# NVlabs/long-video-gan

Hardware: NVIDIA H100
Metric: frames/sec (G+D train step: every convolution and torch_utils.ops call of the forward/backward passes, replayed) (higher is better)
Workload: dtype f32

## Files before the change

include/lvg_ops.h:

```cpp
#ifndef LVG_OPS_H_
#define LVG_OPS_H_

#include <stdint.h>

#ifdef __cplusplus
extern "C" {
#endif

#define LVG_ABI_VERSION 2

#define LVG_OK            0
#define LVG_UNSUPPORTED (-1)
#define LVG_ERR_ARG       1
#define LVG_ERR_CUDA      2

#define LVG_F32 0
#define LVG_F16 1
#define LVG_F64 2

#define LVG_ACT_LINEAR   1
#define LVG_ACT_RELU     2
#define LVG_ACT_LRELU    3
#define LVG_ACT_TANH     4
#define LVG_ACT_SIGMOID  5
// ... 24 lines not shown
                           void* stream);
int64_t lvg_bias_act_codes_bytes(int dtype, int64_t n);

int lvg_upfirdn2d(const void* x, const float* f, void* y, int dtype,
                  const int64_t x_shape[4], const int64_t x_stride[4],
                  const int64_t y_shape[4], const int64_t y_stride[4],
                  int fw, int fh, int64_t f_stride_x, int64_t f_stride_y,
                  int upx, int upy, int downx, int downy, int padx0, int pady0,
                  int flip, float gain, void* stream);

int lvg_upfirdn2d_sep(const void* x, const float* fx, const float* fy, void* y,
                      int dtype, const int64_t x_shape[4], const int64_t x_stride[4],
                      const int64_t y_shape[4], const int64_t y_stride[4],
                      int fw, int fh, int upx, int upy, int downx, int downy,
                      int padx0, int pady0, int flip, float gain, void* stream);

int lvg_filtered_lrelu(const void* x, const float* fu, const float* fd, const void* b,
                       const uint8_t* si, void* y, uint8_t* so, int dtype,
                       const int64_t x_shape[4], const int64_t x_stride[4],
                       const int64_t y_shape[4], const int64_t y_stride[4],
                       int fu_w, int fu_h, int fd_w, int fd_h, int up, int down,
                       int px0, int py0, int s_h, int s_wbytes, int sx, int sy,
                       float gain, float slope, float clamp, int flip,
                       int write_signs, void* stream);

int lvg_filtered_lrelu_supported(int dtype, int fu_w, int fu_h, int fd_w, int fd_h,
                                 int up, int down);

int lvg_filtered_lrelu_act(void* x, const uint8_t* si, uint8_t* so, int dtype,
                           const int64_t x_shape[4], const int64_t x_stride[4],
                           int s_h, int s_wbytes, int sx, int sy, float gain,
                           float slope, float clamp, int write_signs, void* stream);

int lvg_fma(const void* a, const void* b, const void* c, void* out, int dtype,
            int rank, const int64_t shape[6], const int64_t a_stride[6],
            const int64_t b_stride[6], const int64_t c_stride[6], void* stream);

int64_t lvg_convnd_workspace(int dtype, int n, int groups, int cin, int cout, int t, int h, int wd,
                             int kt, int kh, int kw, int pad_t, int pad_h, int pad_w);
int lvg_convnd_fprop(const void* x, const void* w, void* y, int dtype, int n, int groups, int cin, int cout,
                     int t, int h, int wd, int kt, int kh, int kw, int pad_t, int pad_h, int pad_w, int stride,
                     const float* bias, int act, float alpha, float gain, float clamp,
                     void* workspace, int64_t workspace_bytes, void* stream);
int lvg_convnd_dgrad(const void* dy, const void* w, void* dx, int dtype, int n, int groups, int cin, int cout,
                     int t, int h, int wd, int kt, int kh, int kw, int pad_t, int pad_h, int pad_w, int stride,
                     void* workspace, int64_t workspace_bytes, void* stream);
int64_t lvg_convnd_wgrad_workspace(int dtype, int n, int groups, int cin, int cout, int t, int h, int wd,
                                   int kt, int kh, int kw, int pad_t, int pad_h, int pad_w);
int lvg_convnd_wgrad(const void* x, const void* dy, void* dw, int dtype, int n, int groups, int cin, int cout,
                     int t, int h, int wd, int kt, int kh, int kw, int pad_t, int pad_h, int pad_w, int stride,
                     void* workspace, int64_t workspace_bytes, void* stream);
int lvg_convnd_plan(int mode, int dtype, int n, int groups, int cin, int cout, int t, int h, int wd, int kt, int kh, int kw,
                    int pad_t, int pad_h, int pad_w, int stride, int* out, int out_len);
int lvg_convnd_wgrad_plan(int dtype, int n, int groups, int cin, int cout, int t, int h, int wd, int kt, int kh, int kw,
                          int pad_t, int pad_h, int pad_w, int* out, int out_len);
int64_t lvg_convnd_backward_workspace(int dtype, int n, int groups, int cin, int cout, int t, int h, int wd,
                                      int kt, int kh, int kw, int pad_t, int pad_h, int pad_w);
int lvg_convnd_backward(const void* x, const void* dy, const void* w, void* dx, void* dw, int dtype, int n, int groups,
                        int cin, int cout, int t, int h, int wd, int kt, int kh, int kw, int pad_t, int pad_h, int pad_w,
                        int stride, void* workspace, int64_t workspace_bytes, void* stream);

int64_t lvg_modconv_workspace(int dtype, int n, int cin, int cout, int t, int h, int wd, int kt, int kh, int kw,
                              int pad_t, int pad_h, int pad_w);
int lvg_modconv_fprop(const void* x, const void* w, const float* a, const float* d, void* y, int dtype, int n, int cin,
                      int cout, int t, int h, int wd, int kt, int kh, int kw, int pad_t, int pad_h, int pad_w,
                      void* workspace, int64_t workspace_bytes, void* stream);
int lvg_modconv_backward(const void* x, const void* w, const float* a, const float* d, const void* y, const void* dy,
                         void* dx, void* dw, float* da, float* dyy, int dtype, int n, int cin, int cout, int t, int h,
                         int wd, int kt, int kh, int kw, int pad_t, int pad_h, int pad_w, void* workspace,
                         int64_t workspace_bytes, void* stream);

int64_t lvg_fir1d_depthwise_workspace(int groups);
int lvg_fir1d_depthwise(const float* x, const float* w, float* y, int n, int groups, int lin, int k,
                        void* workspace, int64_t workspace_bytes, void* stream);

int lvg_fir3d(const void* x, const float* f, void* y, int dtype, int n, int c, int t_in, int h_in, int w_in, int t_out,
              int h_out, int w_out, int filt_t, int filt_h, int filt_w, int step_t, int step_h, int step_w, int off_t,
              int off_h, int off_w, int fold, void* stream);
int lvg_fir3d_adjoint(const void* x, const float* f, void* y, int dtype, int n, int c, int t_in, int h_in, int w_in,
                      int t_out, int h_out, int w_out, int filt_t, int filt_h, int filt_w, int step_t, int step_h,
                      int step_w, int off_t, int off_h, int off_w, int fold, void* stream);

#define LVG_VIDEO_AUGMENT_LINEAR 1
int64_t lvg_video_augment_workspace(int n, int c, int t_in, int h, int w, int t_out);
int lvg_video_augment(const float* x, const float* params, float* y, void* workspace, int n, int c, int t_in, int h, int w,
                      int t_out, int flags, void* stream);
int lvg_video_augment_adjoint(const float* dy, const float* params, float* dx, void* workspace, int n, int c, int t_in,
                              int h, int w, int t_out, void* stream);

#define LVG_AUGMENT_PIPE_NPAR 23
#define LVG_AUGMENT_PIPE_GEOM 1
#define LVG_AUGMENT_PIPE_LINEAR 2
int64_t lvg_augment_pipe_workspace(int n, int c, int t, int h, int w, int flags);
int lvg_augment_pipe(const float* x, const float* params, const float* filter, int ntaps, const float* noise, float* y, int n,
                     int c, int t, int h, int w, int flags, void* stream);
int lvg_augment_pipe_adjoint(const float* dy, const float* params, const float* filter, int ntaps, float* dx, void* workspace,
                             int n, int c, int t, int h, int w, int flags, void* stream);

int lvg_grad_postprocess(float* g, int64_t n, float scale, float limit, void* stream);

int lvg_adam_step(float* p, float* g, float* m, float* v, float* p_ema, int64_t n, float lr, float beta1, float beta2,
                  float eps, int64_t step, float grad_scale, float grad_limit, int write_grad, float ema_beta, void* stream);

int lvg_lerp(float* a, const float* b, int64_t n, float weight, void* stream);

#ifdef __cplusplus
// ... 4 lines not shown
```

long-video-gan_b200/csrc/conv_igemm.cu:

```cuda

#include <algorithm>
#include <cuda.h>
#include <stdlib.h>
#include <cuda_bf16.h>

#include "common.cuh"
#include "wgmma.cuh"

namespace lvg {
bool pw_supported(int dtype, int groups, int cin, int cout, int kt, int kh, int kw, int pad_t, int pad_h, int pad_w, int stride, int64_t P);
int pw_conv(const float* x, const float* w, float* y, int n, int cin, int cout, int64_t P, int64_t w_sco, int64_t w_sci, cudaStream_t s);
}

namespace lvg {
namespace {

using namespace tc;

constexpr int kBM = 128;
constexpr int kATile = kBM * 16 * 2;
constexpr int kIgemmThreads = 384;
constexpr int kWidths = 16;
constexpr int kMaxStages = 6;
constexpr int kBSlack = 1024;

struct IgemmParams {
    const unsigned char* wp;
    void* y;
    const float* bias;
    int act;
    float alpha, gain, clamp;
    int out_f32;
    int bf16;
    int wgroups, cout, mt, kc;
    int nblk;
    int nimg;
    int lo_blk;
    int to, ho, wo;
    int kt, kh, kw, pad_t, pad_h, pad_w;
    int tt, th, wt, wtb, thb;
    int frame_px;
    int ncols;
    int m64;
    int ncw;
    int a_img;
    int tiles_x, tiles_y, tiles_t;
    int64_t total_tiles;
    int ks;
    int stages;
    int a_resident;
    int a_stage, b_step, b_bytes, b_box, stage_bytes;
    int64_t y_cs;
    int ostride, hos, wos;
    const float* out_scale;
};


__device__ __forceinline__ unsigned short bf16_bits(float v) { return __bfloat16_as_ushort(__float2bfloat16_rn(v)); }
__device__ __forceinline__ float bf16_val(unsigned short b) { return __uint_as_float((uint32_t)b << 16); }

struct PackGeom { int64_t thw_in, thw_out; int ih, iw, oh, ow, dil; const float* scale; };

template <class TIn, bool SPLIT, bool SCALE>
__global__ void __launch_bounds__(256) conv_pack_act_kernel(const TIn* __restrict__ x, uint4* __restrict__ y, int64_t inst, int c,
// ... 546 lines not shown
        const int rc = encode_map(&tm, x8, wd, h, t, inst * g.nblk, wd, (int64_t)h * wd, thw, p.wtb, p.thb, p.tt, 2);
        if (rc) return rc;
    }
    const size_t smem = (size_t)p.stages * p.stage_bytes + 128;
#define LVG_IGEMM_WIDTHS(B, S)                                                                                                     \
    {conv_igemm_kernel<B, 16, S>,  conv_igemm_kernel<B, 32, S>,  conv_igemm_kernel<B, 48, S>,  conv_igemm_kernel<B, 64, S>,        \
     conv_igemm_kernel<B, 80, S>,  conv_igemm_kernel<B, 96, S>,  conv_igemm_kernel<B, 112, S>, conv_igemm_kernel<B, 128, S>,       \
     conv_igemm_kernel<B, 144, S>, conv_igemm_kernel<B, 160, S>, conv_igemm_kernel<B, 176, S>, conv_igemm_kernel<B, 192, S>,       \
     conv_igemm_kernel<B, 208, S>, conv_igemm_kernel<B, 224, S>, conv_igemm_kernel<B, 240, S>, conv_igemm_kernel<B, 256, S>}
    void (*const kerns[2][2][kWidths])(const CUtensorMap, const IgemmParams) = {
        {LVG_IGEMM_WIDTHS(false, false), LVG_IGEMM_WIDTHS(true, false)}, {LVG_IGEMM_WIDTHS(false, true), LVG_IGEMM_WIDTHS(true, true)}};
#undef LVG_IGEMM_WIDTHS
    LVG_REQUIRE(p.ncw % 16 == 0 && p.ncw >= 16 && p.ncw <= 16 * kWidths, "convnd: MMA width %d", p.ncw);
    void (*kern)(const CUtensorMap, const IgemmParams) = kerns[out_scale != nullptr][split][p.ncw / 16 - 1];
    LVG_CUDA(cudaFuncSetAttribute(kern, cudaFuncAttributeMaxDynamicSharedMemorySize, (int)smem));
    const char* cta_env = getenv("LVG_CONV_CTAS");
    const int max_ctas = cta_env ? atoi(cta_env) : num_sms();
    int64_t ctas = p.total_tiles < max_ctas ? p.total_tiles : max_ctas;
    kern<<<(unsigned)ctas, kIgemmThreads, smem, s>>>(tm, p);
    LVG_LAUNCH_CHECK();
    return LVG_OK;
}

bool nd_supported(int dtype, int kt, int kh, int kw)
{
    return (dtype == LVG_F16 || dtype == LVG_F32) && kt >= 1 && kh >= 1 && kw >= 1 && kh * kw <= 9 && kt <= 7;
}

}
}

using namespace lvg;

extern "C" int64_t lvg_convnd_workspace(int dtype, int n, int groups, int cin, int cout, int t, int h, int wd, int kt, int kh, int kw,
                                        int pad_t, int pad_h, int pad_w)
{
    if (!nd_supported(dtype, kt, kh, kw) || n < 1 || groups < 1) return -1;
    const int split = dtype == LVG_F32;
    const int taps = kt * kh * kw;
    const int64_t inst = (int64_t)n * groups;
    const int to = t + 2 * pad_t - kt + 1, ho = h + 2 * pad_h - kh + 1, wo = wd + 2 * pad_w - kw + 1;
    if (to < 1 || ho < 1 || wo < 1) return -1;
    const Geometry a = geometry(split, inst, groups, cin, cout, (int64_t)t * h * wd, taps);
    const Geometry b = geometry(split, inst, groups, cout, cin, (int64_t)to * ho * wo, taps);
    const int64_t fa = a.act_bytes + a.w_bytes, fb = b.act_bytes + b.w_bytes;
    return (fa > fb ? fa : fb) + 1024;
}

extern "C" int lvg_convnd_fprop(const void* x, const void* w, void* y, int dtype, int n, int groups, int cin, int cout, int t, int h, int wd,
                                int kt, int kh, int kw, int pad_t, int pad_h, int pad_w, int stride, const float* bias, int act, float alpha,
                                float gain, float clamp, void* workspace, int64_t workspace_bytes, void* stream)
{
    LVG_REQUIRE(x && w && y, "convnd_fprop: x, w, y must not be NULL");
    if (!bias && act == 0 && gain == 1.f && clamp < 0.f &&
        pw_supported(dtype, groups, cin, cout, kt, kh, kw, pad_t, pad_h, pad_w, stride, (int64_t)t * h * wd))
        return pw_conv((const float*)x, (const float*)w, (float*)y, n, cin, cout, (int64_t)t * h * wd, cin, 1, (cudaStream_t)stream);
    if (!nd_supported(dtype, kt, kh, kw) || n < 1 || pad_t < 0 || pad_h < 0 || pad_w < 0 || stride < 1 || stride > 4) {
        set_error("convnd_fprop: outside the tensor-core kernel's envelope");
        return LVG_UNSUPPORTED;
    }
    const int taps = kt * kh * kw;
    return run_igemm(x, w, y, dtype, n, groups, cin, cout, t, h, wd, kt, kh, kw, pad_t, pad_h, pad_w, (int64_t)cout * cin * taps,
                     (int64_t)cin * taps, taps, 0, bias, act, alpha, gain, clamp, h, wd, 1, stride, nullptr, workspace, workspace_bytes,
                     (cudaStream_t)stream);
}

extern "C" int lvg_convnd_dgrad(const void* dy, const void* w, void* dx, int dtype, int n, int groups, int cin, int cout, int t, int h, int wd,
                                int kt, int kh, int kw, int pad_t, int pad_h, int pad_w, int stride, void* workspace, int64_t workspace_bytes,
                                void* stream)
{
    LVG_REQUIRE(dy && w && dx, "convnd_dgrad: dy, w, dx must not be NULL");
    if (pw_supported(dtype, groups, cin, cout, kt, kh, kw, pad_t, pad_h, pad_w, stride, (int64_t)t * h * wd))
        return pw_conv((const float*)dy, (const float*)w, (float*)dx, n, cout, cin, (int64_t)t * h * wd, 1, cin, (cudaStream_t)stream);
    if (!nd_supported(dtype, kt, kh, kw) || n < 1 || pad_t < 0 || pad_h < 0 || pad_w < 0 || pad_t > kt - 1 || pad_h > kh - 1 || pad_w > kw - 1 ||
        stride < 1 || stride > 4) {
        set_error("convnd_dgrad: outside the tensor-core kernel's envelope");
        return LVG_UNSUPPORTED;
    }
    const int taps = kt * kh * kw;
    const int to = t + 2 * pad_t - kt + 1, ho = h + 2 * pad_h - kh + 1, wo = wd + 2 * pad_w - kw + 1;
    const int hos = (ho - 1) / stride + 1, wos = (wo - 1) / stride + 1;
    return run_igemm(dy, w, dx, dtype, n, groups, cout, cin, to, ho, wo, kt, kh, kw, kt - 1 - pad_t, kh - 1 - pad_h, kw - 1 - pad_w,
                     (int64_t)cout * cin * taps, taps, (int64_t)cin * taps, 1, nullptr, 0, 0.f, 1.f, -1.f, hos, wos, stride, 1, nullptr, workspace,
                     workspace_bytes, (cudaStream_t)stream);
}


namespace lvg {
namespace {

struct WgradV2Params {
    void* dw;
    int out_f32;
    int bf16, split;
    int n, groups, cin, cout;
    int to, ho;
    int kt, kh, kw, pad_t, pad_h, pad_w;
    int nt;
    int nblk_a, nblk_b;
    int lo_a, lo_b;
    int nseg, seg_w[4], seg_x0[4], ps[4];
    int rh;
    int khc;
    int ablk;
    int nsplit;
    int a_bytes, b_bytes, stage_bytes, stages;
    int64_t split_stride;
    int mrows;
    int tail_bytes;
};

struct WgradMaps { CUtensorMap a[4]; CUtensorMap b; };

template <bool BF16, int TAPS, int NT>
__global__ void __launch_bounds__(kIgemmThreads, 1) conv_wgrad_v2_kernel(const __grid_constant__ WgradMaps maps, const WgradV2Params p)
{
    extern __shared__ __align__(128) unsigned char smem_raw[];
    __shared__ uint64_t full_bar[kMaxStages], empty_bar[kMaxStages];
    unsigned char* smem = reinterpret_cast<unsigned char*>((reinterpret_cast<uintptr_t>(smem_raw) + 127) & ~(uintptr_t)127);

    const int warp = threadIdx.x / 32, lane = threadIdx.x % 32;
    const int wg = __shfl_sync(0xffffffffu, (int)threadIdx.x / 128, 0);
    int bx = blockIdx.x;
    const int sp = bx % p.nsplit; bx /= p.nsplit;
    int ky0 = 0;
    if (p.khc == 1) { ky0 = bx % p.kh; bx /= p.kh; }
// ... 278 lines not shown
    {
        const int rc = encode_map(&maps.b, x8, wd, h, t, inst * p.nblk_b, wd, (int64_t)h * wd, thw_b, p.ps[0], p.rh + q.khc - 1, 1, q.nt / 8);
        if (rc) return rc;
    }
    void (*const kern)(const WgradMaps, const WgradV2Params) = wgrad_kernel(q.split, q.khc * kw, q.nt);
    LVG_REQUIRE(kern != nullptr, "convnd_wgrad: no kernel for %d taps x %d columns (split %d)", q.khc * kw, q.nt, q.split);
    LVG_CUDA(cudaFuncSetAttribute(kern, cudaFuncAttributeMaxDynamicSharedMemorySize, (int)smem));
    dim3 grid((unsigned)(q.ntiles * kt * (kh / q.khc) * q.nsplit), (unsigned)q.mt, (unsigned)groups);
    kern<<<grid, kIgemmThreads, smem, s>>>(maps, p);
    LVG_LAUNCH_CHECK();
    if (q.nsplit > 1) {
        int64_t blocks = (q.dw_elems + 255) / 256;
        const int64_t cap = (int64_t)num_sms() * 32;
        if (blocks > cap) blocks = cap;
        if (q.split) conv_wgrad_reduce_kernel<float><<<(unsigned)blocks, 256, 0, s>>>(part, (float*)dw, q.dw_elems, q.nsplit, q.dw_elems);
        else conv_wgrad_reduce_kernel<__half><<<(unsigned)blocks, 256, 0, s>>>(part, (__half*)dw, q.dw_elems, q.nsplit, q.dw_elems);
        LVG_LAUNCH_CHECK();
    }
    return LVG_OK;
}

bool wgrad_in_envelope(int dtype, int n, int groups, int t, int h, int wd, int kt, int kh, int kw, int pad_t, int pad_h, int pad_w, int stride)
{
    const int to = t + 2 * pad_t - kt + 1, ho = h + 2 * pad_h - kh + 1, wo = wd + 2 * pad_w - kw + 1;
    return nd_supported(dtype, kt, kh, kw) && n >= 1 && groups >= 1 && kw <= 3 && pad_t >= 0 && pad_h >= 0 && pad_w >= 0 && to >= 1 && ho >= 1 &&
           wo >= 1 && wo <= 4 * (128 - kw + 1) && stride >= 1 && stride <= 4;
}

}
}

extern "C" int64_t lvg_convnd_wgrad_workspace(int dtype, int n, int groups, int cin, int cout, int t, int h, int wd, int kt, int kh, int kw,
                                              int pad_t, int pad_h, int pad_w)
{
    if (!wgrad_in_envelope(dtype, n, groups, t, h, wd, kt, kh, kw, pad_t, pad_h, pad_w, 1)) return -1;
    const int to = t + 2 * pad_t - kt + 1, ho = h + 2 * pad_h - kh + 1, wo = wd + 2 * pad_w - kw + 1;
    const WgradPlan q = wgrad_plan(dtype, n, groups, cin, cout, t, h, wd, to, ho, wo, kt, kh, kw);
    return q.a_bytes + q.b_bytes + q.part_bytes + 1024;
}

extern "C" int lvg_convnd_wgrad(const void* x, const void* dy, void* dw, int dtype, int n, int groups, int cin, int cout, int t, int h, int wd,
                                int kt, int kh, int kw, int pad_t, int pad_h, int pad_w, int stride, void* workspace, int64_t workspace_bytes,
                                void* stream)
{
    LVG_REQUIRE(x && dy && dw, "convnd_wgrad: x, dy, dw must not be NULL");
    if (!wgrad_in_envelope(dtype, n, groups, t, h, wd, kt, kh, kw, pad_t, pad_h, pad_w, stride)) {
        set_error("convnd_wgrad: outside the tensor-core kernel's envelope");
        return LVG_UNSUPPORTED;
    }
    return run_wgrad(x, dy, dw, dtype, n, groups, cin, cout, t, h, wd, kt, kh, kw, pad_t, pad_h, pad_w, stride, nullptr, workspace, workspace_bytes,
                     (cudaStream_t)stream);
}

extern "C" int lvg_convnd_plan(int mode, int dtype, int n, int groups, int cin, int cout, int t, int h, int wd, int kt, int kh, int kw, int pad_t,
                               int pad_h, int pad_w, int stride, int* out, int out_len)
{
    LVG_REQUIRE(out && out_len >= 48, "convnd_plan: out must hold 48 ints");
    LVG_REQUIRE(mode == 0 || mode == 1, "convnd_plan: mode 0 (forward) or 1 (input gradient)");
    const int taps = kt * kh * kw;
    if (!nd_supported(dtype, kt, kh, kw) || n < 1 || groups < 1 || pad_t < 0 || pad_h < 0 || pad_w < 0 || stride < 1 || stride > 4 ||
        (mode == 1 && (pad_t > kt - 1 || pad_h > kh - 1 || pad_w > kw - 1))) {
        set_error("convnd_plan: outside the tensor-core kernel's envelope");
        return LVG_UNSUPPORTED;
    }
    for (int i = 0; i < out_len; i++) out[i] = 0;
    if (pw_supported(dtype, groups, cin, cout, kt, kh, kw, pad_t, pad_h, pad_w, stride, (int64_t)t * h * wd)) { out[47] = 1; return LVG_OK; }
    IgemmParams p;
    memset(&p, 0, sizeof(p));
    void* dummy = reinterpret_cast<void*>(256);
    g_plan_only = &p;
    int rc;
    if (mode == 0) {
        rc = run_igemm(dummy, dummy, dummy, dtype, n, groups, cin, cout, t, h, wd, kt, kh, kw, pad_t, pad_h, pad_w, (int64_t)cout * cin * taps,
                       (int64_t)cin * taps, taps, 0, nullptr, 0, 0.f, 1.f, -1.f, h, wd, 1, stride, nullptr, nullptr, 0, nullptr);
    } else {
        const int to = t + 2 * pad_t - kt + 1, ho = h + 2 * pad_h - kh + 1, wo = wd + 2 * pad_w - kw + 1;
        if (to < 1 || ho < 1 || wo < 1) { g_plan_only = nullptr; set_error("convnd_plan: empty output"); return LVG_UNSUPPORTED; }
        const int hos = (ho - 1) / stride + 1, wos = (wo - 1) / stride + 1;
        rc = run_igemm(dummy, dummy, dummy, dtype, n, groups, cout, cin, to, ho, wo, kt, kh, kw, kt - 1 - pad_t, kh - 1 - pad_h, kw - 1 - pad_w,
                       (int64_t)cout * cin * taps, taps, (int64_t)cin * taps, 1, nullptr, 0, 0.f, 1.f, -1.f, hos, wos, stride, 1, nullptr, nullptr, 0,
                       nullptr);
    }
    g_plan_only = nullptr;
    if (rc) return rc;
    const int v[48] = {p.wgroups, p.cout, p.mt, p.kc, p.nblk, p.nimg, p.lo_blk, p.to, p.ho, p.wo, p.kt, p.kh, p.kw, p.pad_t, p.pad_h, p.pad_w,
                       p.tt, p.th, p.wt, p.wtb, p.thb, p.frame_px, p.ncols, p.tiles_x, p.tiles_y, p.tiles_t,
                       (int)p.total_tiles, p.ks, p.stages, p.a_resident, p.a_stage, p.b_step, p.b_bytes, p.b_box, p.stage_bytes, p.ostride, p.hos, p.wos,
                       p.m64, p.ncw, 0, 0, 0, 0, 0, 0, 0, 0};
    for (int i = 0; i < 48; i++) out[i] = v[i];
    return LVG_OK;
}

extern "C" int lvg_convnd_wgrad_plan(int dtype, int n, int groups, int cin, int cout, int t, int h, int wd, int kt, int kh, int kw, int pad_t,
                                     int pad_h, int pad_w, int* out, int out_len)
{
    LVG_REQUIRE(out && out_len >= 32, "convnd_wgrad_plan: out must hold 32 ints");
    if (!wgrad_in_envelope(dtype, n, groups, t, h, wd, kt, kh, kw, pad_t, pad_h, pad_w, 1)) {
        set_error("convnd_wgrad_plan: outside the tensor-core kernel's envelope");
        return LVG_UNSUPPORTED;
    }
    const int to = t + 2 * pad_t - kt + 1, ho = h + 2 * pad_h - kh + 1, wo = wd + 2 * pad_w - kw + 1;
    const WgradPlan q = wgrad_plan(dtype, n, groups, cin, cout, t, h, wd, to, ho, wo, kt, kh, kw);
    const int v[32] = {q.split, q.cpad_a, q.cpad_b, q.nt, q.ntiles, q.mt, q.nsplit, q.ablk, q.khc, q.nseg, q.ps, q.rh, q.stages, q.a_stage, q.b_stage,
                       q.stage_bytes, q.tail_bytes, (int)q.smem, q.seg_w[0], q.seg_w[1], q.seg_w[2], q.seg_w[3], q.seg_x0[0], q.seg_x0[1], q.seg_x0[2],
                       q.seg_x0[3], 0, q.mrows, 0, 0, 0, 0};
    for (int i = 0; i < 32; i++) out[i] = v[i];
    return LVG_OK;
}

namespace lvg {
namespace {
bool backward_shares_dy8(int dtype, int n, int groups, int cin, int cout, int t, int h, int wd, int kt, int kh, int kw, int pad_t, int pad_h,
                         int pad_w, int stride)
{
    const int64_t P = (int64_t)t * h * wd;
    if (!env_flag("LVG_CONV_SHARED_DY8", 1)) return false;
    if (pw_supported(dtype, groups, cin, cout, kt, kh, kw, pad_t, pad_h, pad_w, stride, P)) return false;
    return wgrad_cpad_a(cout) == round_up(cout, 16);
}
}
}

extern "C" int64_t lvg_convnd_backward_workspace(int dtype, int n, int groups, int cin, int cout, int t, int h, int wd, int kt, int kh, int kw,
                                                 int pad_t, int pad_h, int pad_w)
{
    const int64_t a = lvg_convnd_workspace(dtype, n, groups, cin, cout, t, h, wd, kt, kh, kw, pad_t, pad_h, pad_w);
    const int64_t b = lvg_convnd_wgrad_workspace(dtype, n, groups, cin, cout, t, h, wd, kt, kh, kw, pad_t, pad_h, pad_w);
    if (a < 0 || b < 0) return -1;
    return a + b + 1024;
}

extern "C" int lvg_convnd_backward(const void* x, const void* dy, const void* w, void* dx, void* dw, int dtype, int n, int groups, int cin, int cout,
                                   int t, int h, int wd, int kt, int kh, int kw, int pad_t, int pad_h, int pad_w, int stride, void* workspace,
                                   int64_t workspace_bytes, void* stream)
{
    LVG_REQUIRE(x && dy && w && dx && dw, "convnd_backward: x, dy, w, dx, dw must not be NULL");
    LVG_REQUIRE(workspace && aligned16(workspace), "convnd_backward: workspace must be 16-byte aligned and not NULL");
    const bool tc_ok = wgrad_in_envelope(dtype, n, groups, t, h, wd, kt, kh, kw, pad_t, pad_h, pad_w, stride) && pad_t <= kt - 1 && pad_h <= kh - 1 &&
                       pad_w <= kw - 1;
    if (!tc_ok || !backward_shares_dy8(dtype, n, groups, cin, cout, t, h, wd, kt, kh, kw, pad_t, pad_h, pad_w, stride)) {
        const int rc = lvg_convnd_dgrad(dy, w, dx, dtype, n, groups, cin, cout, t, h, wd, kt, kh, kw, pad_t, pad_h, pad_w, stride, workspace,
                                        workspace_bytes, stream);
        if (rc) return rc;
        return lvg_convnd_wgrad(x, dy, dw, dtype, n, groups, cin, cout, t, h, wd, kt, kh, kw, pad_t, pad_h, pad_w, stride, workspace, workspace_bytes,
                                stream);
    }
    cudaStream_t s = (cudaStream_t)stream;
    const int split = dtype == LVG_F32 ? 1 : 0;
    const int taps = kt * kh * kw;
    const int to = t + 2 * pad_t - kt + 1, ho = h + 2 * pad_h - kh + 1, wo = wd + 2 * pad_w - kw + 1;
    const int hos = (ho - 1) / stride + 1, wos = (wo - 1) / stride + 1;
    const int64_t inst = (int64_t)n * groups;
    const Geometry gd = geometry(split, inst, groups, cout, cin, (int64_t)to * ho * wo, taps);
    const int64_t dy8_room = ((gd.act_bytes + 255) / 256) * 256;
    const int64_t wp_room = ((gd.w_bytes + 255) / 256) * 256 + 256;
    LVG_REQUIRE(workspace_bytes >= dy8_room + wp_room, "convnd_backward: workspace too small");
    unsigned char* dy8 = reinterpret_cast<unsigned char*>(workspace);
    unsigned char* rest = dy8 + dy8_room;
    int rc = pack_act(dy, dy8, split, inst, cout, gd.cblk, to, hos, wos, ho, wo, stride, s);
    if (rc) return rc;
    rc = run_igemm(dy, w, dx, dtype, n, groups, cout, cin, to, ho, wo, kt, kh, kw, kt - 1 - pad_t, kh - 1 - pad_h, kw - 1 - pad_w,
                   (int64_t)cout * cin * taps, taps, (int64_t)cin * taps, 1, nullptr, 0, 0.f, 1.f, -1.f, hos, wos, stride, 1, dy8, rest, wp_room, s);
    if (rc) return rc;
    return run_wgrad(x, dy, dw, dtype, n, groups, cin, cout, t, h, wd, kt, kh, kw, pad_t, pad_h, pad_w, stride, dy8, rest,
                     workspace_bytes - dy8_room, s);
}


namespace lvg {
namespace {
// ... 155 lines not shown
```

long-video-gan_b200/torch_utils/custom_ops.py:

```python
import ctypes
import math
import os

import torch

verbosity = 'brief'

_LIB_NAME = 'liblvg_ops.so'
_lib = None
_plugins = {}

_c_void_p = ctypes.c_void_p
_c_int = ctypes.c_int
_c_i64 = ctypes.c_int64
_c_float = ctypes.c_float
_I64x4 = ctypes.c_int64 * 4
_I64x6 = ctypes.c_int64 * 6

_DTYPE_CODE = {torch.float32: 0, torch.float16: 1, torch.float64: 2}

_SIGNATURES = {
    'lvg_abi_version': (_c_int, []),
    'lvg_last_error': (ctypes.c_char_p, []),
    'lvg_build_info': (ctypes.c_char_p, []),
    'lvg_launch_count': (_c_i64, []),
    'lvg_grad_postprocess': (_c_int, [_c_void_p, _c_i64, _c_float, _c_float, _c_void_p]),
    'lvg_adam_step': (_c_int, [_c_void_p] * 5 + [_c_i64] + [_c_float] * 4 + [_c_i64, _c_float, _c_float, _c_int, _c_float, _c_void_p]),
    'lvg_lerp': (_c_int, [_c_void_p, _c_void_p, _c_i64, _c_float, _c_void_p]),
    'lvg_bias_act': (_c_int, [_c_void_p] * 6 + [_c_int, _c_i64, _c_i64, _c_i64, _c_int, _c_int, _c_float, _c_float, _c_float, _c_void_p]),
    'lvg_bias_act_grad_db': (_c_int, [_c_void_p] * 6 + [_c_int, _c_i64, _c_i64, _c_i64, _c_int, _c_float, _c_float, _c_float, _c_void_p]),
    'lvg_bias_act_fwd_codes': (_c_int, [_c_void_p] * 4 + [_c_int, _c_i64, _c_i64, _c_i64, _c_int, _c_float, _c_float, _c_float, _c_void_p]),
    'lvg_bias_act_codes_bytes': (_c_i64, [_c_int, _c_i64]),
    'lvg_bias_act_bwd_codes': (_c_int, [_c_void_p] * 4 + [_c_int, _c_i64, _c_i64, _c_i64, _c_int, _c_float, _c_float, _c_float, _c_void_p]),
    'lvg_upfirdn2d': (_c_int, [_c_void_p, _c_void_p, _c_void_p, _c_int, _I64x4, _I64x4, _I64x4, _I64x4, _c_int, _c_int, _c_i64, _c_i64]
                      + [_c_int] * 7 + [_c_float, _c_void_p]),
    'lvg_upfirdn2d_sep': (_c_int, [_c_void_p] * 4 + [_c_int, _I64x4, _I64x4, _I64x4, _I64x4] + [_c_int] * 9 + [_c_float, _c_void_p]),
    'lvg_filtered_lrelu': (_c_int, [_c_void_p] * 7 + [_c_int, _I64x4, _I64x4, _I64x4, _I64x4] + [_c_int] * 12
                           + [_c_float, _c_float, _c_float, _c_int, _c_int, _c_void_p]),
    'lvg_filtered_lrelu_supported': (_c_int, [_c_int] * 7),
    'lvg_filtered_lrelu_act': (_c_int, [_c_void_p] * 3 + [_c_int, _I64x4, _I64x4] + [_c_int] * 4 + [_c_float] * 3 + [_c_int, _c_void_p]),
    'lvg_fma': (_c_int, [_c_void_p] * 4 + [_c_int, _c_int, _I64x6, _I64x6, _I64x6, _I64x6, _c_void_p]),
    'lvg_fir1d_depthwise_workspace': (_c_i64, [_c_int]),
    'lvg_fir1d_depthwise': (_c_int, [_c_void_p] * 3 + [_c_int] * 4 + [_c_void_p, _c_i64, _c_void_p]),
    'lvg_convnd_workspace': (_c_i64, [_c_int] * 14),
    'lvg_convnd_fprop': (_c_int, [_c_void_p] * 3 + [_c_int] * 15 + [_c_void_p, _c_int, _c_float, _c_float, _c_float, _c_void_p, _c_i64, _c_void_p]),
    'lvg_convnd_dgrad': (_c_int, [_c_void_p] * 3 + [_c_int] * 15 + [_c_void_p, _c_i64, _c_void_p]),
    'lvg_convnd_wgrad_workspace': (_c_i64, [_c_int] * 14),
    'lvg_convnd_wgrad': (_c_int, [_c_void_p] * 3 + [_c_int] * 15 + [_c_void_p, _c_i64, _c_void_p]),
    'lvg_convnd_plan': (_c_int, [_c_int] * 16 + [ctypes.POINTER(_c_int), _c_int]),
    'lvg_convnd_wgrad_plan': (_c_int, [_c_int] * 14 + [ctypes.POINTER(_c_int), _c_int]),
    'lvg_convnd_backward_workspace': (_c_i64, [_c_int] * 14),
    'lvg_convnd_backward': (_c_int, [_c_void_p] * 5 + [_c_int] * 15 + [_c_void_p, _c_i64, _c_void_p]),
    'lvg_modconv_workspace': (_c_i64, [_c_int] * 13),
    'lvg_modconv_fprop': (_c_int, [_c_void_p] * 5 + [_c_int] * 13 + [_c_void_p, _c_i64, _c_void_p]),
    'lvg_modconv_backward': (_c_int, [_c_void_p] * 10 + [_c_int] * 13 + [_c_void_p, _c_i64, _c_void_p]),
    'lvg_fir3d': (_c_int, [_c_void_p] * 3 + [_c_int] * 19 + [_c_void_p]),
    'lvg_fir3d_adjoint': (_c_int, [_c_void_p] * 3 + [_c_int] * 19 + [_c_void_p]),
    'lvg_video_augment_workspace': (_c_i64, [_c_int] * 6),
    'lvg_video_augment': (_c_int, [_c_void_p] * 4 + [_c_int] * 7 + [_c_void_p]),
    'lvg_video_augment_adjoint': (_c_int, [_c_void_p] * 4 + [_c_int] * 6 + [_c_void_p]),
    'lvg_augment_pipe_workspace': (_c_i64, [_c_int] * 6),
    'lvg_augment_pipe': (_c_int, [_c_void_p] * 3 + [_c_int] + [_c_void_p] * 2 + [_c_int] * 6 + [_c_void_p]),
    'lvg_augment_pipe_adjoint': (_c_int, [_c_void_p] * 3 + [_c_int] + [_c_void_p] * 2 + [_c_int] * 6 + [_c_void_p]),
}

LVG_UNSUPPORTED = -1


def library_path():
    return os.path.join(os.path.dirname(os.path.dirname(os.path.abspath(__file__))), _LIB_NAME)


def load_library():
    global _lib
    if _lib is None:
        path = os.environ.get('LVG_OPS_LIBRARY', library_path())
        if not os.path.isfile(path):
            raise RuntimeError(
                f'{_LIB_NAME} not found at {path}: build it with `python -c "import __graft_entry__ as g; g.build()"` '
                f'or `make -C long-video-gan_b200/csrc`. There is no fallback for CUDA tensors.')
        lib = ctypes.CDLL(path)
        for name, (restype, argtypes) in _SIGNATURES.items():
            fn = getattr(lib, name)
            fn.restype = restype
            fn.argtypes = argtypes
        if lib.lvg_abi_version() != 2:
            raise RuntimeError(f'{path}: unexpected ABI version {lib.lvg_abi_version()}')
        _lib = lib
    return _lib


def exported_symbols():
    return sorted(_SIGNATURES)


def launch_count():
    return int(load_library().lvg_launch_count())


def _check(rc, what):
    if rc > 0:
        raise RuntimeError(f'{what}: {_lib.lvg_last_error().decode()}')
    return rc
# ... 358 lines not shown


class ConvNdPlugin:

    def __init__(self, lib):
        self._lib = lib
        self._ws = {}

    @staticmethod
    def _pad3(padding, nd):
        p = list(padding) if isinstance(padding, (list, tuple)) else [padding] * nd
        return [0] * (3 - nd) + [int(v) for v in p]

    def supported(self, x, w, stride, padding, dilation, groups):
        return x.is_cuda and self._in_envelope(tuple(x.shape), tuple(w.shape), x.dtype if w.dtype == x.dtype else None, stride, padding,
                                               dilation, groups)

    @staticmethod
    def _in_envelope(x_shape, w_shape, dtype, stride, padding, dilation, groups):
        if not (dtype in (torch.float16, torch.float32) and len(x_shape) == len(w_shape) and len(x_shape) in (3, 4, 5)):
            return False
        nd = len(x_shape) - 2
        as_t = lambda v: tuple(v) if isinstance(v, (list, tuple)) else (v,) * nd
        st = as_t(stride)
        if as_t(dilation) != (1,) * nd or len(set(st[-2:])) != 1 or not (1 <= st[-1] <= 4) or (nd == 3 and st[0] != 1) or (nd == 1 and st[0] != 1):
            return False
        sp = [1] * (3 - nd) + list(x_shape[2:])
        k = [1] * (3 - nd) + list(w_shape[2:])
        pad = ConvNdPlugin._pad3(padding, nd)
        if k[1] * k[2] > 9 or k[0] > 7 or k[2] > 3 or min(pad) < 0 or any(p > kk - 1 for p, kk in zip(pad, k)):
            return False
        if x_shape[1] != w_shape[1] * groups or w_shape[0] % groups != 0 or x_shape[0] * groups > 65535 or math.prod(x_shape) == 0:
            return False
        out = [s + 2 * p - kk + 1 for s, p, kk in zip(sp, pad, k)]
        return min(out) >= 1 and out[2] <= 4 * (128 - k[2] + 1)

    def _workspace(self, device, need):
        if need < 0:
            raise RuntimeError('convnd: configuration outside the tensor-core kernel envelope')
        buf = self._ws.get(device)
        if buf is None or buf.numel() < need:
            buf = torch.empty(max(int(need), 1 << 22), dtype=torch.uint8, device=device)
            self._ws[device] = buf
        return buf

    def _args(self, x_shape, w_shape, padding, groups, dtype):
        nd = len(x_shape) - 2
        sp = [1] * (3 - nd) + list(x_shape[2:])
        k = [1] * (3 - nd) + list(w_shape[2:])
        pad = self._pad3(padding, nd)
        code = 1 if dtype == torch.float16 else 0
        return [code, x_shape[0], groups, w_shape[1], w_shape[0] // groups] + sp + k + pad, sp, k, pad

    def fprop(self, x, w, padding, groups, bias=None, act=0, alpha=0.2, gain=1.0, clamp=-1.0, stride=1):
        x, w = x.contiguous(), w.contiguous()
        a, sp, k, pad = self._args(tuple(x.shape), tuple(w.shape), padding, groups, x.dtype)
        st3 = [1, stride, stride] if x.ndim >= 4 else [1, 1, 1]
        out_sp = [(s + 2 * p - kk) // q + 1 for s, p, kk, q in zip(sp, pad, k, st3)][3 - (x.ndim - 2):]
        y = torch.empty([x.shape[0], w.shape[0]] + out_sp, dtype=x.dtype, device=x.device)
        ws = self._workspace(x.device, self._lib.lvg_convnd_workspace(*a))
        if bias is not None:
            bias = bias.to(torch.float32).contiguous()
        with _DeviceGuard(x):
            rc = _check(self._lib.lvg_convnd_fprop(_ptr(x), _ptr(w), _ptr(y), *a, int(stride), _ptr(bias), int(act), float(alpha), float(gain),
                                                   float(clamp), _ptr(ws), ws.numel(), _stream(x)), 'convnd_fprop')
        if rc == LVG_UNSUPPORTED:
            raise RuntimeError('convnd_fprop: ' + self._lib.lvg_last_error().decode())
        return y

    def dgrad(self, dy, w, x_shape, padding, groups, stride=1):
        dy, w = dy.contiguous(), w.contiguous()
        a, sp, k, pad = self._args(tuple(x_shape), tuple(w.shape), padding, groups, dy.dtype)
        dx = torch.empty(list(x_shape), dtype=dy.dtype, device=dy.device)
        ws = self._workspace(dy.device, self._lib.lvg_convnd_workspace(*a))
        with _DeviceGuard(dy):
            rc = _check(self._lib.lvg_convnd_dgrad(_ptr(dy), _ptr(w), _ptr(dx), *a, int(stride), _ptr(ws), ws.numel(), _stream(dy)), 'convnd_dgrad')
        if rc == LVG_UNSUPPORTED:
            raise RuntimeError('convnd_dgrad: ' + self._lib.lvg_last_error().decode())
        return dx

    def fir1d_depthwise(self, x, w):
        x, w = x.contiguous(), w.contiguous()
        n, g, lin = x.shape
        k = w.shape[2]
        y = torch.empty([n, g, lin - k + 1], dtype=x.dtype, device=x.device)
        ws = torch.empty([g + 4], dtype=torch.int32, device=x.device)
        with _DeviceGuard(x):
            _check(self._lib.lvg_fir1d_depthwise(_ptr(x), _ptr(w), _ptr(y), n, g, lin, k, _ptr(ws), ws.numel() * 4, _stream(x)), 'fir1d_depthwise')
        return y

    def wgrad(self, x, dy, w_shape, padding, groups, stride=1):
        x, dy = x.contiguous(), dy.contiguous()
        a, sp, k, pad = self._args(tuple(x.shape), tuple(w_shape), padding, groups, x.dtype)
        dw = torch.empty(list(w_shape), dtype=x.dtype, device=x.device)
        ws = self._workspace(x.device, self._lib.lvg_convnd_wgrad_workspace(*a))
        with _DeviceGuard(x):
            rc = _check(self._lib.lvg_convnd_wgrad(_ptr(x), _ptr(dy), _ptr(dw), *a, int(stride), _ptr(ws), ws.numel(), _stream(x)), 'convnd_wgrad')
        if rc == LVG_UNSUPPORTED:
            raise RuntimeError('convnd_wgrad: ' + self._lib.lvg_last_error().decode())
        return dw

    def backward(self, x, dy, w, padding, groups, stride=1):
        x, dy, w = x.contiguous(), dy.contiguous(), w.contiguous()
        a, sp, k, pad = self._args(tuple(x.shape), tuple(w.shape), padding, groups, x.dtype)
        dx = torch.empty_like(x)
        dw = torch.empty_like(w)
# ... 172 lines not shown
```

Baseline: 2052.

## Add dedicated TMA+WGMMA pointwise conv kernel and route 1x1 fprop/dgrad to it

Adds a specialized warp-specialized kernel for 1x1 convolutions. It TMA-loads raw activations and converts them in shared memory to bf16 hi/lo split (f32) or f16 tiles, then issues WGMMA against prepacked weights. A new route function sends 1x1 fprop/dgrad shapes that the small SIMT path does not take to this kernel instead of the general implicit-GEMM engine. The goal is to skip the generic engine's separate activation packing pass and im2col overhead. The cost is a per-call weight pack launch and a tensor map encode, and the risk that the engine already handled these shapes well.

Measured after the change: 2141, median of 6. 1.04x the previous value.

```diff
diff --git a/include/lvg_ops.h b/include/lvg_ops.h
--- a/include/lvg_ops.h
+++ b/include/lvg_ops.h
@@ -100,6 +100,8 @@
                      void* workspace, int64_t workspace_bytes, void* stream);
 int lvg_convnd_plan(int mode, int dtype, int n, int groups, int cin, int cout, int t, int h, int wd, int kt, int kh, int kw,
                     int pad_t, int pad_h, int pad_w, int stride, int* out, int out_len);
+int lvg_convnd_route(int mode, int dtype, int n, int groups, int cin, int cout, int t, int h, int wd, int kt, int kh, int kw,
+                     int pad_t, int pad_h, int pad_w, int stride, int epilogue);
 int lvg_convnd_wgrad_plan(int dtype, int n, int groups, int cin, int cout, int t, int h, int wd, int kt, int kh, int kw,
                           int pad_t, int pad_h, int pad_w, int* out, int out_len);
 int64_t lvg_convnd_backward_workspace(int dtype, int n, int groups, int cin, int cout, int t, int h, int wd,
diff --git a/long-video-gan_b200/csrc/conv_igemm.cu b/long-video-gan_b200/csrc/conv_igemm.cu
--- a/long-video-gan_b200/csrc/conv_igemm.cu
+++ b/long-video-gan_b200/csrc/conv_igemm.cu
@@ -10,6 +10,9 @@
 namespace lvg {
 bool pw_supported(int dtype, int groups, int cin, int cout, int kt, int kh, int kw, int pad_t, int pad_h, int pad_w, int stride, int64_t P);
 int pw_conv(const float* x, const float* w, float* y, int n, int cin, int cout, int64_t P, int64_t w_sco, int64_t w_sci, cudaStream_t s);
+bool pw_tc_supported(int dtype, int groups, int cin, int cout, int kt, int kh, int kw, int pad_t, int pad_h, int pad_w, int stride, int64_t P);
+int pw_tc_conv(const void* x, const void* w, void* y, int dtype, int n, int ck, int cm, int64_t P, int64_t w_sm, int64_t w_sk, void* workspace,
+               int64_t workspace_bytes, cudaStream_t s);
 }
 
 namespace lvg {
@@ -662,9 +665,11 @@
                                 float gain, float clamp, void* workspace, int64_t workspace_bytes, void* stream)
 {
     LVG_REQUIRE(x && w && y, "convnd_fprop: x, w, y must not be NULL");
-    if (!bias && act == 0 && gain == 1.f && clamp < 0.f &&
-        pw_supported(dtype, groups, cin, cout, kt, kh, kw, pad_t, pad_h, pad_w, stride, (int64_t)t * h * wd))
-        return pw_conv((const float*)x, (const float*)w, (float*)y, n, cin, cout, (int64_t)t * h * wd, cin, 1, (cudaStream_t)stream);
+    const int route = lvg_convnd_route(0, dtype, n, groups, cin, cout, t, h, wd, kt, kh, kw, pad_t, pad_h, pad_w, stride,
+                                       bias || act != 0 || gain != 1.f || clamp >= 0.f);
+    if (route == 1) return pw_conv((const float*)x, (const float*)w, (float*)y, n, cin, cout, (int64_t)t * h * wd, cin, 1, (cudaStream_t)stream);
+    if (route == 2 && aligned16(x) && aligned16(y))
+        return pw_tc_conv(x, w, y, dtype, n, cin, cout, (int64_t)t * h * wd, cin, 1, workspace, workspace_bytes, (cudaStream_t)stream);
     if (!nd_supported(dtype, kt, kh, kw) || n < 1 || pad_t < 0 || pad_h < 0 || pad_w < 0 || stride < 1 || stride > 4) {
         set_error("convnd_fprop: outside the tensor-core kernel's envelope");
         return LVG_UNSUPPORTED;
@@ -680,8 +685,10 @@
                                 void* stream)
 {
     LVG_REQUIRE(dy && w && dx, "convnd_dgrad: dy, w, dx must not be NULL");
-    if (pw_supported(dtype, groups, cin, cout, kt, kh, kw, pad_t, pad_h, pad_w, stride, (int64_t)t * h * wd))
-        return pw_conv((const float*)dy, (const float*)w, (float*)dx, n, cout, cin, (int64_t)t * h * wd, 1, cin, (cudaStream_t)stream);
+    const int route = lvg_convnd_route(1, dtype, n, groups, cin, cout, t, h, wd, kt, kh, kw, pad_t, pad_h, pad_w, stride, 0);
+    if (route == 1) return pw_conv((const float*)dy, (const float*)w, (float*)dx, n, cout, cin, (int64_t)t * h * wd, 1, cin, (cudaStream_t)stream);
+    if (route == 2 && aligned16(dy) && aligned16(dx))
+        return pw_tc_conv(dy, w, dx, dtype, n, cout, cin, (int64_t)t * h * wd, 1, cin, workspace, workspace_bytes, (cudaStream_t)stream);
     if (!nd_supported(dtype, kt, kh, kw) || n < 1 || pad_t < 0 || pad_h < 0 || pad_w < 0 || pad_t > kt - 1 || pad_h > kh - 1 || pad_w > kw - 1 ||
         stride < 1 || stride > 4) {
         set_error("convnd_dgrad: outside the tensor-core kernel's envelope");
@@ -1066,6 +1073,22 @@
                      (cudaStream_t)stream);
 }
 
+extern "C" int lvg_convnd_route(int mode, int dtype, int n, int groups, int cin, int cout, int t, int h, int wd, int kt, int kh, int kw, int pad_t,
+                                int pad_h, int pad_w, int stride, int epilogue)
+{
+    if (mode < 0 || mode > 2 || n < 1 || groups < 1) return LVG_UNSUPPORTED;
+    if (mode == 2) return wgrad_in_envelope(dtype, n, groups, t, h, wd, kt, kh, kw, pad_t, pad_h, pad_w, stride) ? 0 : LVG_UNSUPPORTED;
+    const int64_t P = (int64_t)t * h * wd;
+    if (mode == 1 || !epilogue) {
+        if (pw_supported(dtype, groups, cin, cout, kt, kh, kw, pad_t, pad_h, pad_w, stride, P)) return 1;
+        if (pw_tc_supported(dtype, groups, cin, cout, kt, kh, kw, pad_t, pad_h, pad_w, stride, P)) return 2;
+    }
+    if (!nd_supported(dtype, kt, kh, kw) || pad_t < 0 || pad_h < 0 || pad_w < 0 || stride < 1 || stride > 4 ||
+        (mode == 1 && (pad_t > kt - 1 || pad_h > kh - 1 || pad_w > kw - 1)))
+        return LVG_UNSUPPORTED;
+    return 0;
+}
+
 extern "C" int lvg_convnd_plan(int mode, int dtype, int n, int groups, int cin, int cout, int t, int h, int wd, int kt, int kh, int kw, int pad_t,
                                int pad_h, int pad_w, int stride, int* out, int out_len)
 {
@@ -1130,6 +1153,7 @@
     const int64_t P = (int64_t)t * h * wd;
     if (!env_flag("LVG_CONV_SHARED_DY8", 1)) return false;
     if (pw_supported(dtype, groups, cin, cout, kt, kh, kw, pad_t, pad_h, pad_w, stride, P)) return false;
+    if (pw_tc_supported(dtype, groups, cin, cout, kt, kh, kw, pad_t, pad_h, pad_w, stride, P)) return false;
     return wgrad_cpad_a(cout) == round_up(cout, 16);
 }
 }
diff --git a/long-video-gan_b200/csrc/conv_pw_tc.cu b/long-video-gan_b200/csrc/conv_pw_tc.cu
--- /dev/null
+++ b/long-video-gan_b200/csrc/conv_pw_tc.cu
@@ -0,0 +1,302 @@
+#include <cuda.h>
+#include <stdlib.h>
+#include <cuda_bf16.h>
+
+#include "common.cuh"
+#include "wgmma.cuh"
+
+namespace lvg {
+namespace {
+
+using namespace tc;
+
+constexpr int kPtThreads = 384;
+constexpr int kPtNP = 128;
+constexpr int kPtKS = 2;
+constexpr int kPtStages = 4;
+constexpr int kPtSBO = 272;
+constexpr int kPtBImg = (kPtNP / 8) * kPtSBO;
+
+struct PwTcParams {
+    const unsigned char* wp;
+    void* y;
+    int cout, mt, kc, nimg, a_img, m64;
+    int64_t P;
+    int ptiles;
+    int64_t total_tiles;
+    int raw_bytes;
+    int w_step;
+    int w_off, b_off, stage_bytes;
+};
+
+__device__ __forceinline__ unsigned short pt_bf16_bits(float v) { return __bfloat16_as_ushort(__float2bfloat16_rn(v)); }
+__device__ __forceinline__ float pt_bf16_val(unsigned short b) { return __uint_as_float((uint32_t)b << 16); }
+
+__device__ __forceinline__ void tma_load_3d(void* dst, const CUtensorMap* map, int c0, int c1, int c2, uint64_t* bar)
+{
+    asm volatile("cp.async.bulk.tensor.3d.shared::cluster.global.tile.mbarrier::complete_tx::bytes [%0], [%1, {%2, %3, %4}], [%5];"
+                 ::"r"(smem_u32(dst)), "l"(reinterpret_cast<uint64_t>(map)), "r"(c0), "r"(c1), "r"(c2), "r"(smem_u32(bar))
+                 : "memory");
+}
+
+__device__ __forceinline__ void consumer_bar_sync() { asm volatile("bar.sync 1, 256;" ::: "memory"); }
+
+template <class TW, bool SPLIT>
+__global__ void __launch_bounds__(256) conv_pw_tc_pack_w_kernel(const TW* __restrict__ w, unsigned char* __restrict__ wp, int m_total, int k_total,
+                                                                 int64_t sm, int64_t sk, int mt, int kc, int rows)
+{
+    constexpr int NIMG = SPLIT ? 2 : 1;
+    const int img = rows * 32;
+    const int total = mt * kc * 2 * rows;
+    for (int i = blockIdx.x * blockDim.x + threadIdx.x; i < total; i += gridDim.x * blockDim.x) {
+        const int r = i % rows;
+        const int k8 = (i / rows) % 2;
+        const int kci = (i / (2 * rows)) % kc;
+        const int mti = i / (2 * rows * kc);
+        const int m = mti * rows + r;
+        alignas(16) unsigned short v[8], vlo[8];
+#pragma unroll
+        for (int j = 0; j < 8; j++) {
+            const int k = kci * 16 + k8 * 8 + j;
+            const bool ok = m < m_total && k < k_total;
+            if constexpr (SPLIT) {
+                const float f = ok ? __ldg(reinterpret_cast<const float*>(w) + m * sm + k * sk) : 0.f;
+                v[j] = pt_bf16_bits(f);
+                vlo[j] = pt_bf16_bits(f - pt_bf16_val(v[j]));
+            } else {
+                v[j] = ok ? __half_as_ushort(__ldg(reinterpret_cast<const __half*>(w) + m * sm + k * sk)) : (unsigned short)0;
+            }
+        }
+        unsigned char* d = wp + ((int64_t)(mti * kc + kci) * NIMG) * img + k8 * (img / 2) + r * 16;
+        *reinterpret_cast<uint4*>(d) = *reinterpret_cast<const uint4*>(v);
+        if constexpr (SPLIT) *reinterpret_cast<uint4*>(d + img) = *reinterpret_cast<const uint4*>(vlo);
+    }
+}
+
+template <bool BF16, int NW>
+__global__ void __launch_bounds__(kPtThreads, 1) conv_pw_tc_kernel(const __grid_constant__ CUtensorMap tmx, const PwTcParams p)
+{
+    extern __shared__ __align__(128) unsigned char smem_raw[];
+    __shared__ uint64_t full_bar[kPtStages], empty_bar[kPtStages];
+    unsigned char* smem = reinterpret_cast<unsigned char*>((reinterpret_cast<uintptr_t>(smem_raw) + 127) & ~(uintptr_t)127);
+
+    const int warp = threadIdx.x / 32, lane = threadIdx.x % 32;
+    const int wg = __shfl_sync(0xffffffffu, (int)threadIdx.x / 128, 0);
+    const int kchunks = (p.kc + kPtKS - 1) / kPtKS;
+
+    if (threadIdx.x == 0) {
+        for (int s = 0; s < kPtStages; s++) { mbar_init(&full_bar[s], 1); mbar_init(&empty_bar[s], 2); }
+        fence_barrier_init();
+    }
+    __syncthreads();
+
+    if (wg == 0) {
+        if (warp == 0 && elect_one()) {
+            int it = 0;
+            for (int64_t L = blockIdx.x; L < p.total_tiles; L += gridDim.x) {
+                const int mti = (int)(L % p.mt);
+                const int64_t r = L / p.mt;
+                const int pt = (int)(r % p.ptiles);
+                const int n = (int)(r / p.ptiles);
+                const unsigned char* wpm = p.wp + (int64_t)mti * p.kc * p.w_step;
+                for (int kcix = 0; kcix < kchunks; kcix++, it++) {
+                    const int s = it % kPtStages;
+                    if (it >= kPtStages) mbar_wait(&empty_bar[s], (uint32_t)((it / kPtStages - 1) & 1));
+                    unsigned char* st = smem + (size_t)s * p.stage_bytes;
+                    const int k0 = kcix * kPtKS;
+                    const int nks = min(kPtKS, p.kc - k0);
+                    const uint32_t wb = (uint32_t)(nks * p.w_step);
+                    mbar_expect_tx(&full_bar[s], wb + (uint32_t)p.raw_bytes);
+                    bulk_copy_g2s(st + p.w_off, wpm + (int64_t)k0 * p.w_step, wb, &full_bar[s]);
+                    tma_load_3d(st, &tmx, pt * kPtNP, k0 * 16, n, &full_bar[s]);
+                }
+            }
+        }
+    } else {
+        const int cw = wg - 1;
+        const int ctid = threadIdx.x - 128;
+        const int tid = threadIdx.x % 128, wq = tid / 32;
+        const uint32_t a_hi = desc_hi(128), b_hi = desc_hi(kPtSBO);
+        const uint32_t a_lo_img = (uint32_t)p.a_img >> 4, b_lo_img = (uint32_t)kPtBImg >> 4;
+        const uint32_t a_row0 = p.m64 ? 0u : (uint32_t)cw * 1024u;
+        const int col0 = p.m64 ? cw * NW : 0;
+        int it = 0;
+        for (int64_t L = blockIdx.x; L < p.total_tiles; L += gridDim.x) {
+            const int mti = (int)(L % p.mt);
+            const int64_t r = L / p.mt;
+            const int pt = (int)(r % p.ptiles);
+            const int n = (int)(r / p.ptiles);
+            float acc[NW / 2];
+#pragma unroll
+            for (int i = 0; i < NW / 2; i++) acc[i] = 0.f;
+            int prev = -1;
+            for (int kcix = 0; kcix < kchunks; kcix++, it++) {
+                const int s = it % kPtStages;
+                const int nks = min(kPtKS, p.kc - kcix * kPtKS);
+                unsigned char* st = smem + (size_t)s * p.stage_bytes;
+                unsigned char* bimg = st + p.b_off;
+                mbar_wait(&full_bar[s], (uint32_t)((it / kPtStages) & 1));
+                if constexpr (BF16) {
+                    const float* raw = reinterpret_cast<const float*>(st);
+                    for (int i = ctid; i < nks * 16 * (kPtNP / 4); i += 256) {
+                        const int q = i % (kPtNP / 4), k = i / (kPtNP / 4);
+                        const float4 v = *reinterpret_cast<const float4*>(raw + k * kPtNP + 4 * q);
+                        const float f[4] = {v.x, v.y, v.z, v.w};
+                        alignas(8) unsigned short hi[4], lo[4];
+#pragma unroll
+                        for (int e = 0; e < 4; e++) {
+                            hi[e] = pt_bf16_bits(f[e]);
+                            lo[e] = pt_bf16_bits(f[e] - pt_bf16_val(hi[e]));
+                        }
+                        const int j = k / 16, kk = k % 16;
+                        unsigned char* d = bimg + j * (2 * kPtBImg) + (q / 2) * kPtSBO + (kk / 8) * 128 + (kk % 8) * 16 + (q % 2) * 8;
+                        *reinterpret_cast<uint2*>(d) = *reinterpret_cast<const uint2*>(hi);
+                        *reinterpret_cast<uint2*>(d + kPtBImg) = *reinterpret_cast<const uint2*>(lo);
+                    }
+                } else {
+                    const uint4* raw = reinterpret_cast<const uint4*>(st);
+                    for (int i = ctid; i < nks * 16 * (kPtNP / 8); i += 256) {
+                        const int g = i % (kPtNP / 8), k = i / (kPtNP / 8);
+                        const int j = k / 16, kk = k % 16;
+                        *reinterpret_cast<uint4*>(bimg + j * kPtBImg + g * kPtSBO + (kk / 8) * 128 + (kk % 8) * 16) = raw[k * (kPtNP / 8) + g];
+                    }
+                }
+                fence_proxy_async();
+                consumer_bar_sync();
+                wgmma_fence();
+                const uint32_t sa = smem_u32(st + p.w_off), sb = smem_u32(bimg) + (uint32_t)(col0 / 8) * kPtSBO;
+                for (int j = 0; j < nks; j++) {
+                    const uint32_t a_lo = desc_lo(sa + (uint32_t)(j * p.w_step) + a_row0, (uint32_t)p.a_img / 2);
+                    const uint32_t b_lo = desc_lo(sb + (uint32_t)(j * p.nimg * kPtBImg), 128);
+                    wgmma_m64nNk16<BF16, NW, 0, 1>(acc, a_lo, a_hi, b_lo, b_hi);
+                    if constexpr (BF16) {
+                        wgmma_m64nNk16<BF16, NW, 0, 1>(acc, a_lo, a_hi, b_lo + b_lo_img, b_hi);
+                        wgmma_m64nNk16<BF16, NW, 0, 1>(acc, a_lo + a_lo_img, a_hi, b_lo, b_hi);
+                    }
+                }
+                wgmma_commit();
+                wgmma_wait<1>();
+                mbar_arrive_if(&empty_bar[prev >= 0 ? prev : 0], prev >= 0 && tid == 0);
+                prev = s;
+            }
+            wgmma_wait<0>();
+            mbar_arrive_if(&empty_bar[prev], tid == 0);
+
+            const int64_t p0 = (int64_t)pt * kPtNP;
+#pragma unroll
+            for (int h = 0; h < 2; h++) {
+                const int row = wq * 16 + lane / 4 + 8 * h;
+                const int co = p.m64 ? row : mti * 128 + cw * 64 + row;
+                if (co >= p.cout) continue;
+                const int64_t base = ((int64_t)n * p.cout + co) * p.P + p0;
+#pragma unroll
+                for (int j = 0; j < NW / 8; j++) {
+                    const int col = col0 + j * 8 + 2 * (lane % 4);
+                    if (p0 + col >= p.P) continue;
+                    const float v0 = acc[4 * j + 2 * h], v1 = acc[4 * j + 2 * h + 1];
+                    if constexpr (BF16) *reinterpret_cast<float2*>(reinterpret_cast<float*>(p.y) + base + col) = make_float2(v0, v1);
+                    else *reinterpret_cast<__half2*>(reinterpret_cast<__half*>(p.y) + base + col) = __floats2half2_rn(v0, v1);
+                }
+            }
+        }
+    }
+}
+
+typedef CUresult (*PtEncodeFn)(CUtensorMap*, CUtensorMapDataType, cuuint32_t, void*, const cuuint64_t*, const cuuint64_t*, const cuuint32_t*,
+                               const cuuint32_t*, CUtensorMapInterleave, CUtensorMapSwizzle, CUtensorMapL2promotion, CUtensorMapFloatOOBfill);
+
+PtEncodeFn pt_encode_fn()
+{
+    static PtEncodeFn fn = [] {
+        void* f = nullptr;
+        cudaDriverEntryPointQueryResult q;
+        if (cudaGetDriverEntryPoint("cuTensorMapEncodeTiled", &f, cudaEnableDefault, &q) != cudaSuccess || q != cudaDriverEntryPointSuccess) f = nullptr;
+        return reinterpret_cast<PtEncodeFn>(f);
+    }();
+    return fn;
+}
+
+struct PwTcGeom { int kc, mt, m64, nimg, a_img; int64_t w_bytes; };
+
+PwTcGeom pw_tc_geometry(int split, int ck, int cm)
+{
+    PwTcGeom g;
+    g.kc = (ck + 15) / 16;
+    g.m64 = cm <= 64 ? 1 : 0;
+    g.mt = g.m64 ? 1 : (cm + 127) / 128;
+    g.nimg = split ? 2 : 1;
+    g.a_img = g.m64 ? 2048 : 4096;
+    g.w_bytes = (int64_t)g.mt * g.kc * g.nimg * g.a_img;
+    return g;
+}
+
+}
+
+bool pw_tc_supported(int dtype, int groups, int cin, int cout, int kt, int kh, int kw, int pad_t, int pad_h, int pad_w, int stride, int64_t P)
+{
+    const char* e = getenv("LVG_CONV_PW_TC");
+    if (e && e[0] == '0') return false;
+    const int64_t align = dtype == LVG_F32 ? 4 : 8;
+    return (dtype == LVG_F32 || dtype == LVG_F16) && groups == 1 && kt == 1 && kh == 1 && kw == 1 && pad_t == 0 && pad_h == 0 && pad_w == 0 &&
+           stride == 1 && cin >= 1 && cout >= 1 && P >= align && P % align == 0 && P / kPtNP < (1ll << 30);
+}
+
+int64_t pw_tc_workspace(int dtype, int ck, int cm) { return pw_tc_geometry(dtype == LVG_F32, ck, cm).w_bytes + 256; }
+
+int pw_tc_conv(const void* x, const void* w, void* y, int dtype, int n, int ck, int cm, int64_t P, int64_t w_sm, int64_t w_sk, void* workspace,
+               int64_t workspace_bytes, cudaStream_t s)
+{
+    const int split = dtype == LVG_F32 ? 1 : 0;
+    const int es = split ? 4 : 2;
+    const PwTcGeom g = pw_tc_geometry(split, ck, cm);
+    LVG_REQUIRE(aligned16(x) && aligned16(y), "pointwise conv: tensors must be 16-byte aligned");
+    LVG_REQUIRE(workspace && aligned16(workspace) && workspace_bytes >= g.w_bytes, "pointwise conv: workspace too small");
+    PtEncodeFn enc = pt_encode_fn();
+    LVG_REQUIRE(enc != nullptr, "pointwise conv: cuTensorMapEncodeTiled is not available from this driver");
+
+    unsigned char* wp = reinterpret_cast<unsigned char*>(workspace);
+    {
+        const int rows = g.m64 ? 64 : 128;
+        const int total = g.mt * g.kc * 2 * rows;
+        const int blocks = (total + 255) / 256;
+        if (split) conv_pw_tc_pack_w_kernel<float, true><<<blocks, 256, 0, s>>>((const float*)w, wp, cm, ck, w_sm, w_sk, g.mt, g.kc, rows);
+        else conv_pw_tc_pack_w_kernel<__half, false><<<blocks, 256, 0, s>>>((const __half*)w, wp, cm, ck, w_sm, w_sk, g.mt, g.kc, rows);
+        LVG_LAUNCH_CHECK();
+    }
+
+    CUtensorMap tm;
+    {
+        const cuuint64_t dims[3] = {(cuuint64_t)P, (cuuint64_t)ck, (cuuint64_t)n};
+        const cuuint64_t strides[2] = {(cuuint64_t)P * es, (cuuint64_t)P * ck * es};
+        const cuuint32_t box[3] = {(cuuint32_t)kPtNP, (cuuint32_t)(kPtKS * 16), 1};
+        const cuuint32_t estr[3] = {1, 1, 1};
+        const CUresult r = enc(&tm, split ? CU_TENSOR_MAP_DATA_TYPE_UINT32 : CU_TENSOR_MAP_DATA_TYPE_UINT16, 3, const_cast<void*>(x), dims, strides,
+                               box, estr, CU_TENSOR_MAP_INTERLEAVE_NONE, CU_TENSOR_MAP_SWIZZLE_NONE, CU_TENSOR_MAP_L2_PROMOTION_L2_256B,
+                               CU_TENSOR_MAP_FLOAT_OOB_FILL_NONE);
+        LVG_REQUIRE(r == CUDA_SUCCESS, "pointwise conv: cuTensorMapEncodeTiled failed (%d)", (int)r);
+    }
+
+    PwTcParams p;
+    memset(&p, 0, sizeof(p));
+    p.wp = wp; p.y = y;
+    p.cout = cm; p.mt = g.mt; p.kc = g.kc; p.nimg = g.nimg; p.a_img = g.a_img; p.m64 = g.m64;
+    p.P = P;
+    p.ptiles = (int)((P + kPtNP - 1) / kPtNP);
+    p.total_tiles = (int64_t)n * p.ptiles * g.mt;
+    p.raw_bytes = kPtKS * 16 * kPtNP * es;
+    p.w_step = g.nimg * g.a_img;
+    p.w_off = p.raw_bytes;
+    p.b_off = p.w_off + kPtKS * p.w_step;
+    p.stage_bytes = p.b_off + kPtKS * g.nimg * kPtBImg;
+    const size_t smem = (size_t)kPtStages * p.stage_bytes + 128;
+
+    void (*kern)(const CUtensorMap, const PwTcParams) =
+        split ? (g.m64 ? conv_pw_tc_kernel<true, 64> : conv_pw_tc_kernel<true, 128>) : (g.m64 ? conv_pw_tc_kernel<false, 64> : conv_pw_tc_kernel<false, 128>);
+    LVG_CUDA(cudaFuncSetAttribute(kern, cudaFuncAttributeMaxDynamicSharedMemorySize, (int)smem));
+    const int64_t ctas = p.total_tiles < num_sms() ? p.total_tiles : num_sms();
+    kern<<<(unsigned)ctas, kPtThreads, smem, s>>>(tm, p);
+    LVG_LAUNCH_CHECK();
+    return LVG_OK;
+}
+
+}
diff --git a/long-video-gan_b200/torch_utils/custom_ops.py b/long-video-gan_b200/torch_utils/custom_ops.py
--- a/long-video-gan_b200/torch_utils/custom_ops.py
+++ b/long-video-gan_b200/torch_utils/custom_ops.py
@@ -49,6 +49,7 @@
     'lvg_convnd_wgrad': (_c_int, [_c_void_p] * 3 + [_c_int] * 15 + [_c_void_p, _c_i64, _c_void_p]),
     'lvg_convnd_plan': (_c_int, [_c_int] * 16 + [ctypes.POINTER(_c_int), _c_int]),
     'lvg_convnd_wgrad_plan': (_c_int, [_c_int] * 14 + [ctypes.POINTER(_c_int), _c_int]),
+    'lvg_convnd_route': (_c_int, [_c_int] * 17),
     'lvg_convnd_backward_workspace': (_c_i64, [_c_int] * 14),
     'lvg_convnd_backward': (_c_int, [_c_void_p] * 5 + [_c_int] * 15 + [_c_void_p, _c_i64, _c_void_p]),
     'lvg_modconv_workspace': (_c_i64, [_c_int] * 13),
@@ -513,6 +514,13 @@
         code = 1 if dtype == torch.float16 else 0
         return [code, x_shape[0], groups, w_shape[1], w_shape[0] // groups] + sp + k + pad, sp, k, pad
 
+    ROUTES = ('engine', 'simt', 'pointwise_wgmma')
+
+    def route(self, mode, x_shape, w_shape, padding, groups, dtype, stride=1, epilogue=False):
+        a, _, _, _ = self._args(tuple(x_shape), tuple(w_shape), padding, groups, dtype)
+        r = self._lib.lvg_convnd_route(('fprop', 'dgrad', 'wgrad').index(mode), *a, int(stride), int(bool(epilogue)))
+        return None if r < 0 else self.ROUTES[r]
+
     def fprop(self, x, w, padding, groups, bias=None, act=0, alpha=0.2, gain=1.0, clamp=-1.0, stride=1):
         x, w = x.contiguous(), w.contiguous()
         a, sp, k, pad = self._args(tuple(x.shape), tuple(w.shape), padding, groups, x.dtype)
```
